# apachepinot/pinot

Hardware: AMD Instinct MI355X
Metric: rows scanned/sec, 1B-row segment filter+groupby (3 predicates, SUM/MAX GROUP BY g1) (higher is better)
Workload: dtype int64; 1 GPU; 1 segment(s) x 1000000000 rows, one per GPU; SELECT g1, SUM(m), MAX(m) FROM gpuBench WHERE c_inv1 IN (0,1,2,3) AND c_inv2 IN (0,1) AND r_int BETWEEN 250000 AND 749999 GROUP BY g1 ORDER BY g1 LIMIT 1000; query=cfg3, parallelism=segment-per-gpu x1, merge=none (1 segment), entries_scanned_in_filter=249990290

## Files before the change

pinot_amd/csrc/pg_kernels_spec.hip:

```cpp
#define PG_WAVES_PER_BLOCK 12
#define PG_KERNEL template <int PG_NOT_INSTANTIATED> static
#include "pg_kernels.hip"

#define SPEC_LOADERS 4
#ifndef SPEC_TILES
#define SPEC_TILES 2
#endif
#ifndef SPEC_SETS
#define SPEC_SETS 2
#endif
#define SPEC_CONSUMERS 8
#define SPEC_OFF_LIN 0u
#define SPEC_OFF_RNG 256u
#define SPEC_OFF_VAL (256u + 2048u)
#define SPEC_OFF_G0 (256u + 2048u + 8192u)
extern "C" const int pg_spec_waves_per_block = PG_WAVES_PER_BLOCK;
extern "C" int pg_spec_stage_bytes(int bits0, int bits1) { return SPEC_TILES * (((int)SPEC_OFF_G0 + bits0 * 256 + 16 + (bits1 > 0 ? bits1 * 256 + 16 : 0) + 15) & ~15); }

DEVFN void spec_barrier() {
  __builtin_amdgcn_fence(__ATOMIC_RELEASE, "workgroup", "local");
  __builtin_amdgcn_s_barrier();
  __builtin_amdgcn_fence(__ATOMIC_ACQUIRE, "workgroup", "local");
}

template <typename T> DEVFN const GAS T* spec_sgpr_ptr(const void* ptr) {
  const uint64_t v = (uint64_t)ptr;
  const uint32_t lo = (uint32_t)__builtin_amdgcn_readfirstlane((int)(uint32_t)v), hi = (uint32_t)__builtin_amdgcn_readfirstlane((int)(uint32_t)(v >> 32));
  return (const GAS T*)(((uint64_t)hi << 32) | (uint64_t)lo);
}

template <int W> struct SpecCol;
template <> struct SpecCol<0> {};
template <> struct SpecCol<32> { u32x4 r[2]; };
template <> struct SpecCol<24> { u32x4 lo; u32x2 hi; };
template <> struct SpecCol<16> { u32x4 lo; };
template <> struct SpecCol<8> { u32x2 hi; };
constexpr uint32_t spec_img_tile_bytes(int W) { return (uint32_t)(PG_WAVE_DOCS / 8) * (uint32_t)W; }
template <int W> DEVFN void spec_load(SpecCol<W>& c, const uint8_t* base, int wt, int w, int lane) {
  if constexpr (W == 32) {
#pragma unroll
    for (int s = 0; s < 2; s++) {
      const uint8_t* row = base + (size_t)wt * (PG_WAVE_DOCS * 4) + (size_t)(4 * s + w) * 1024u;
      c.r[s] = ldnt((const GAS u32x4*)(spec_sgpr_ptr<uint8_t>(row) + (uint32_t)lane * 16u));
    }
  } else if constexpr (W != 0) {
    const uint8_t* tile = base + (size_t)wt * spec_img_tile_bytes(W);
    if constexpr (W >= 16) c.lo = ldnt((const GAS u32x4*)(spec_sgpr_ptr<uint8_t>(tile + (size_t)w * 1024u) + (uint32_t)lane * 16u));
    if constexpr (W != 16) c.hi = ldnt((const GAS u32x2*)(spec_sgpr_ptr<uint8_t>(tile + (W == 24 ? 4096u : 0u) + (size_t)w * 512u) + (uint32_t)lane * 8u));
  }
}
template <int W> DEVFN void spec_unpack(const SpecCol<W>& c, uint32_t (&a)[4], uint32_t (&b)[4]) {
  if constexpr (W == 32) {
    a[0] = bswap32(c.r[0].x); a[1] = bswap32(c.r[0].y); a[2] = bswap32(c.r[0].z); a[3] = bswap32(c.r[0].w);
    b[0] = bswap32(c.r[1].x); b[1] = bswap32(c.r[1].y); b[2] = bswap32(c.r[1].z); b[3] = bswap32(c.r[1].w);
  } else if constexpr (W == 24) {
    a[0] = __builtin_amdgcn_perm(c.hi.x, c.lo.x, 0x0c040100u); a[1] = __builtin_amdgcn_perm(c.hi.x, c.lo.x, 0x0c050302u);
    a[2] = __builtin_amdgcn_perm(c.hi.x, c.lo.y, 0x0c060100u); a[3] = __builtin_amdgcn_perm(c.hi.x, c.lo.y, 0x0c070302u);
    b[0] = __builtin_amdgcn_perm(c.hi.y, c.lo.z, 0x0c040100u); b[1] = __builtin_amdgcn_perm(c.hi.y, c.lo.z, 0x0c050302u);
    b[2] = __builtin_amdgcn_perm(c.hi.y, c.lo.w, 0x0c060100u); b[3] = __builtin_amdgcn_perm(c.hi.y, c.lo.w, 0x0c070302u);
  } else if constexpr (W == 16) {
    a[0] = c.lo.x & 0xFFFFu; a[1] = c.lo.x >> 16; a[2] = c.lo.y & 0xFFFFu; a[3] = c.lo.y >> 16;
    b[0] = c.lo.z & 0xFFFFu; b[1] = c.lo.z >> 16; b[2] = c.lo.w & 0xFFFFu; b[3] = c.lo.w >> 16;
  } else if constexpr (W == 8) {
#pragma unroll
    for (int e = 0; e < 4; e++) { a[e] = (c.hi.x >> (8 * e)) & 0xFFu; b[e] = (c.hi.y >> (8 * e)) & 0xFFu; }
  }
}
template <int SW, int VW> struct SpecTile {
  SpecCol<SW> scan;
  SpecCol<VW> val;
  u32x4 grp;
};
template <int SW, int VW> struct SpecStage { SpecTile<SW, VW> tile[SPEC_TILES]; uint32_t post[8]; uint32_t tail; };
template <int NG> struct SpecQuad {
  uint32_t lin, rng;
  u32x4 val;
  uint32_t win[NG][2];
};

template <int W> struct SpecWidth { static constexpr int value = W; };
template <int NG, bool HAS_INDEX, bool HAS_SCAN, bool HAS_TAIL = false, bool NARROW = false>
__device__ __forceinline__ void spec_body(const PgQueryPlan& p) {
  extern __shared__ __attribute__((aligned(16))) uint64_t smem[];
  __shared__ uint32_t s_stat[PG_MAX_STATS];
  const int t = threadIdx.x;
  const int lane = t & 63;
  const int wave = uniform(t >> 6);
  int64_t* lds_table = reinterpret_cast<int64_t*>(smem);
  if (t < PG_MAX_STATS) s_stat[t] = 0;
  const uint32_t real_slots = (uint32_t)p.n_groups * (uint32_t)p.replicas;
  const uint32_t table_slots = real_slots + 64u;
  for (int o = 0; o < p.n_ops; o++) {
    const int64_t ident = pg_acc_identity(p.ops[o].fn, p.ops[o].is_float);
    for (uint32_t i = t; i < table_slots; i += PG_BLOCK) lds_table[(size_t)o * table_slots + i] = ident;
  }
  const uint32_t bits0 = (uint32_t)p.gcols[0].bits, bits1 = NG > 1 ? (uint32_t)p.gcols[NG - 1].bits : 0u;
  const uint32_t off_g1 = SPEC_OFF_G0 + bits0 * 256u + 16u;
  const uint32_t tile_bytes = (off_g1 + (NG > 1 ? bits1 * 256u + 16u : 0u) + 15u) & ~15u;
  const uint32_t stage_bytes = tile_bytes * SPEC_TILES;
  uint8_t* stage0 = reinterpret_cast<uint8_t*>(smem) + (((size_t)p.n_ops * table_slots * 8u + 15u) & ~(size_t)15u);
  const CAS PgScanLeaf& L = cptr(p.scans)[HAS_SCAN ? p.fast_scan : 0];
  const int grid = (int)gridDim.x;
  const int n_mine = (int)blockIdx.x < p.n_wtiles ? (p.n_wtiles - (int)blockIdx.x + grid - 1) / grid : 0;
  const int n_stages = (n_mine + SPEC_TILES - 1) / SPEC_TILES;
  __syncthreads();

  if (wave < SPEC_LOADERS) {
    const int w = wave;
    const uint8_t* const xdata = p.srcs[p.pipe_src].data;
    const uint8_t* const simg = NARROW ? p.spec_simg : nullptr;
    const uint8_t* const vimg = NARROW ? p.spec_vimg : nullptr;
    const uint32_t img_slo = NARROW ? p.spec_slo : 0u, img_sspan = NARROW ? p.spec_sspan : 0u, img_vmin = NARROW ? (uint32_t)p.spec_vmin : 0u;
    const bool img_sempty = NARROW && p.spec_sempty != 0;
    const int ggi = (w >> 1) < NG ? (w >> 1) : 0;
    const uint8_t* const gdata = p.gcols[ggi].data;
    const uint32_t gbits = (uint32_t)p.gcols[ggi].bits;
    const uint32_t goff = (uint32_t)(w & 1) * 1024u + (uint32_t)lane * 16u;
    const uint32_t geff = (w >> 1) < NG && goff < gbits * 256u ? goff : 0u;
    const uint8_t* dense_ptr[8];
    int dense_group[8];
#pragma unroll
    for (int j = 0; j < 8; j++) { dense_ptr[j] = HAS_INDEX ? p.dense_ptr[j] : nullptr; dense_group[j] = HAS_INDEX ? p.dense_group[j] : 0; }
    const int dense_groups = p.dense_groups, dense_excl = p.dense_excl;
    const uint8_t* const pipe_tail = HAS_TAIL ? p.pipe_tail : nullptr;
    const int num_docs = p.num_docs;
    const bool scan_pushed = p.fast_scan_pushed != 0;
   auto loaders = [&](auto scan_w, auto val_w) __attribute__((always_inline)) {
    constexpr int SW = HAS_SCAN ? decltype(scan_w)::value : 0, VW = decltype(val_w)::value;
    const RangeI32 r32 = !HAS_SCAN ? RangeI32{0, 0u, false} : (SW == 32 ? make_range_i32(L.lo, L.hi) : RangeI32{(int32_t)img_slo, img_sspan, img_sempty});
    const uint8_t* sdata = !HAS_SCAN ? nullptr : (SW == 32 ? L.data : simg);
    const uint8_t* vdata = VW == 32 ? xdata : vimg;
    const uint32_t vmin = VW == 32 ? 0u : img_vmin;
    uint32_t ld_cand = 0;
    auto issue = [&](int sidx, SpecStage<SW, VW>& st) __attribute__((always_inline)) {
#pragma unroll
      for (int tt = 0; tt < SPEC_TILES; tt++) {
        const int i = sidx * SPEC_TILES + tt;
        const int wt = (int)blockIdx.x + (i < n_mine ? i : n_mine - 1) * grid;
        SpecTile<SW, VW>& tl = st.tile[tt];
        __builtin_amdgcn_sched_barrier(0);
        spec_load<SW>(tl.scan, sdata, wt, w, lane);
        spec_load<VW>(tl.val, vdata, wt, w, lane);
        __builtin_amdgcn_sched_barrier(0);
        {
          const uint8_t* base = gdata + (size_t)wt * (size_t)(PG_WAVE_DOCS / 8) * (size_t)gbits;
          tl.grp = ldnt((const GAS u32x4*)(spec_sgpr_ptr<uint8_t>(base) + geff));
        }
        __builtin_amdgcn_sched_barrier(0);
      }
      if (HAS_INDEX) {
        const int i = sidx * SPEC_TILES + (w % SPEC_TILES);
        const int wt = (int)blockIdx.x + (i < n_mine ? i : n_mine - 1) * grid;
#pragma unroll
        for (int j = 0; j < 8; j++) st.post[j] = *(const GAS uint32_t*)(spec_sgpr_ptr<uint8_t>(dense_ptr[j] + (size_t)wt * 256u) + (uint32_t)lane * 4u);
        __builtin_amdgcn_sched_barrier(0);
      }
      if (HAS_TAIL) {
        const int i = sidx * SPEC_TILES + (w % SPEC_TILES);
        const int wt = (int)blockIdx.x + (i < n_mine ? i : n_mine - 1) * grid;
        st.tail = *(const GAS uint32_t*)(spec_sgpr_ptr<uint8_t>(pipe_tail + (size_t)wt * 256u) + (uint32_t)lane * 4u);
        __builtin_amdgcn_sched_barrier(0);
      }
    };
    auto publish = [&](uint8_t* stage, const SpecStage<SW, VW>& st) __attribute__((always_inline)) {
#ifdef PG_SPEC_NO_PUBLISH
      {
        uint32_t acc = 0;
#pragma unroll
        for (int tt = 0; tt < SPEC_TILES; tt++) {
          uint32_t a[4] = {0u, 0u, 0u, 0u}, b[4] = {0u, 0u, 0u, 0u};
          spec_unpack<SW>(st.tile[tt].scan, a, b); acc += a[0] ^ b[3];
          spec_unpack<VW>(st.tile[tt].val, a, b); acc += a[0] ^ b[3];
          acc += st.tile[tt].grp.x;
        }
        if (acc == 0x12345678u) *reinterpret_cast<uint32_t*>(stage) = acc;
        return;
      }
#endif
#pragma unroll
      for (int tt = 0; tt < SPEC_TILES; tt++) {
        uint8_t* buf = stage + (uint32_t)tt * tile_bytes;
        const SpecTile<SW, VW>& tl = st.tile[tt];
        if (HAS_SCAN) {
          uint32_t q[2][4];
          spec_unpack<SW>(tl.scan, q[0], q[1]);
#pragma unroll
          for (int s = 0; s < 2; s++) {
            uint32_t m = (uint32_t)in_range_i32(r32, (int32_t)q[s][0]) | ((uint32_t)in_range_i32(r32, (int32_t)q[s][1]) << 1) |
                         ((uint32_t)in_range_i32(r32, (int32_t)q[s][2]) << 2) | ((uint32_t)in_range_i32(r32, (int32_t)q[s][3]) << 3);
            m = r32.empty ? 0u : m;
            *reinterpret_cast<uint32_t*>(buf + SPEC_OFF_RNG + (uint32_t)(4 * s + w) * 256u + (uint32_t)lane * 4u) = m;
          }
        }
        {
          uint32_t q[2][4];
          spec_unpack<VW>(tl.val, q[0], q[1]);
#pragma unroll
          for (int s = 0; s < 2; s++) {
            u32x4 v;
            v.x = q[s][0] + vmin; v.y = q[s][1] + vmin; v.z = q[s][2] + vmin; v.w = q[s][3] + vmin;
            *reinterpret_cast<u32x4*>(buf + SPEC_OFF_VAL + (uint32_t)(4 * s + w) * 1024u + (uint32_t)lane * 16u) = v;
          }
        }
        *reinterpret_cast<u32x4*>(buf + (ggi == 0 ? SPEC_OFF_G0 : off_g1) + geff) = tl.grp;
      }
    };
    auto publish_lin = [&](uint8_t* stage, const SpecStage<SW, VW>& st, int sidx) __attribute__((always_inline)) {
      if (w >= SPEC_TILES) return;
      const int i = sidx * SPEC_TILES + w;
      const int wt = (int)blockIdx.x + i * grid;
      const int64_t rem = i < n_mine ? (int64_t)num_docs - (int64_t)wt * PG_WAVE_DOCS : 0;
      const int32_t n_valid = rem >= PG_WAVE_DOCS ? PG_WAVE_DOCS : (rem > 0 ? (int32_t)rem : 0);
      uint32_t lin = valid_lin_mask(n_valid, lane);
      if (HAS_INDEX) {
        uint32_t grp[4] = {0u, 0u, 0u, 0u};
#pragma unroll
        for (int j = 0; j < 8; j++) {
          const int gj = dense_group[j];
#pragma unroll
          for (int k = 0; k < 4; k++) grp[k] |= gj == k ? st.post[j] : 0u;
        }
#pragma unroll
        for (int k = 0; k < 4; k++)
          if (k < dense_groups) lin &= ((dense_excl >> k) & 1) ? ~grp[k] : grp[k];
      }
      *reinterpret_cast<uint32_t*>(stage + (uint32_t)w * tile_bytes + SPEC_OFF_LIN + (uint32_t)lane * 4u) = HAS_TAIL ? lin & st.tail : lin;
      ld_cand += (uint32_t)__popc(lin);
    };
    constexpr int SETS = HAS_SCAN ? SPEC_SETS : 2 * SPEC_SETS;
    SpecStage<SW, VW> st[SETS];
    auto buf_of = [&](int sg) __attribute__((always_inline)) { return stage0 + (uint32_t)(sg & 1) * stage_bytes; };
    if (n_stages > 0) {
#pragma unroll
      for (int k = 0; k < SETS; k++) issue(k, st[k]);
    }
    int s = 0;
    for (; s + SETS - 1 < n_stages; s += SETS) {
#pragma unroll
      for (int k = 0; k < SETS; k++) {
        publish(buf_of(s + k), st[k]);
        publish_lin(buf_of(s + k), st[k], s + k);
        issue(s + k + SETS, st[k]);
        spec_barrier();
      }
    }
#pragma unroll
    for (int k = 0; k < SETS - 1; k++)
      if (s + k < n_stages) {
        publish(buf_of(s + k), st[k]);
        publish_lin(buf_of(s + k), st[k], s + k);
        spec_barrier();
      }
    const uint32_t csum = wave_sum_u32(ld_cand);
    if (HAS_SCAN && !scan_pushed && lane == 0 && csum) atomicAdd(&s_stat[L.stat_slot], csum);
   };
    if constexpr (!NARROW) {
      loaders(SpecWidth<32>{}, SpecWidth<32>{});
    } else {
      const int sb = uniform(p.spec_sbits), vb = uniform(p.spec_vbits);
      auto with_scan = [&](auto scan_w) __attribute__((always_inline)) {
        switch (vb) {
          case 8: loaders(scan_w, SpecWidth<8>{}); break;
          case 16: loaders(scan_w, SpecWidth<16>{}); break;
          case 24: loaders(scan_w, SpecWidth<24>{}); break;
          default: loaders(scan_w, SpecWidth<32>{}); break;
        }
      };
      switch (sb) {
        case 8: with_scan(SpecWidth<8>{}); break;
        case 16: with_scan(SpecWidth<16>{}); break;
        case 24: with_scan(SpecWidth<24>{}); break;
        default: with_scan(SpecWidth<32>{}); break;
      }
    }
  } else {
    const int c = wave - SPEC_LOADERS;
    const uint32_t R = (uint32_t)p.replicas;
    const uint32_t rep = (uint32_t)t & (R - 1u);
    const uint32_t stride = table_slots;
    const uint32_t trash_slot = real_slots + (uint32_t)lane;
    const uint32_t q = (uint32_t)c * 64u + (uint32_t)lane;
    const uint32_t nib = ((uint32_t)lane & 7u) * 4u;
    uint32_t my_matched = 0;
    const int n_ops = uniform(p.n_ops);
    uint64_t ops_code = 0;
    for (int o = 0; o < n_ops; o++) {
      const PgAccOp op = p.ops[uniform(o)];
      ops_code |= (uint64_t)(op.src < 0 ? 0u : (op.fn == PG_ACC_SUM ? 1u : (op.fn == PG_ACC_MIN ? 2u : 3u))) << (2 * o);
    }
    ops_code = ((uint64_t)(uint32_t)uniform((int)(uint32_t)(ops_code >> 32)) << 32) | (uint64_t)(uint32_t)uniform((int)(uint32_t)ops_code);
    const int has_out_words = uniform(p.out_words != nullptr ? 1 : 0);
    auto fetch = [&](const uint8_t* buf, SpecQuad<NG>& d) __attribute__((always_inline)) {
      d.lin = *reinterpret_cast<const uint32_t*>(buf + SPEC_OFF_LIN + (q >> 3) * 4u);
      d.rng = HAS_SCAN ? *reinterpret_cast<const uint32_t*>(buf + SPEC_OFF_RNG + q * 4u) : 0xFu;
      d.val = *reinterpret_cast<const u32x4*>(buf + SPEC_OFF_VAL + q * 16u);
#pragma unroll
      for (int gi = 0; gi < NG; gi++) {
        const uint32_t di = __umul24(4u * q, (uint32_t)p.gcols[gi].bits) >> 5;
        const uint32_t* win = reinterpret_cast<const uint32_t*>(buf + (gi == 0 ? SPEC_OFF_G0 : off_g1)) + di;
        d.win[gi][0] = win[0]; d.win[gi][1] = win[1];
      }
    };
    auto aggregate = [&](const SpecQuad<NG> (&d)[SPEC_TILES], int sidx) __attribute__((always_inline)) {
      constexpr int ND = 4 * SPEC_TILES;
      uint32_t slot[ND];
      int32_t v[ND];
#pragma unroll
      for (int tt = 0; tt < SPEC_TILES; tt++) {
        const int i = sidx * SPEC_TILES + tt;
        const uint32_t cand = (d[tt].lin >> nib) & 0xFu;
        const uint32_t m = d[tt].rng & cand;
        my_matched += (uint32_t)__popc(m);
        if (has_out_words && i < n_mine) {
          const int wt = (int)blockIdx.x + i * grid;
          const uint32_t word = or_reduce8(m << nib);
          if ((lane & 7) == 0) reinterpret_cast<uint32_t*>(p.out_words)[(int64_t)wt * 64 + (int64_t)(q >> 3)] = word;
        }
#ifndef PG_SPEC_NO_TABLE
#pragma unroll
        for (int e = 0; e < 4; e++) slot[4 * tt + e] = rep;
#pragma unroll
        for (int gi = 0; gi < NG; gi++) {
          const PgGroupCol& gc = p.gcols[gi];
          const uint32_t bits = (uint32_t)gc.bits, mask = (1u << gc.bits) - 1u;
          const uint32_t mult = (uint32_t)gc.mult * R;
          uint32_t dv[4];
          decode_packed_quad<true>(d[tt].win[gi], q, bits, mask, dv);
#pragma unroll
          for (int e = 0; e < 4; e++) slot[4 * tt + e] += __umul24(dv[e], mult);
        }
#pragma unroll
        for (int e = 0; e < 4; e++) slot[4 * tt + e] = ((m >> e) & 1u) ? slot[4 * tt + e] : trash_slot;
        v[4 * tt + 0] = (int32_t)d[tt].val.x; v[4 * tt + 1] = (int32_t)d[tt].val.y; v[4 * tt + 2] = (int32_t)d[tt].val.z; v[4 * tt + 3] = (int32_t)d[tt].val.w;
#endif
      }
#ifdef PG_SPEC_NO_TABLE
      return;
#endif
      for (int o = 0; o < n_ops; o++) {
        const uint32_t code = (uint32_t)(ops_code >> (2 * o)) & 3u;
        int64_t* base = lds_table + (size_t)o * stride;
        if (code == 0u) {
#pragma unroll
          for (int e = 0; e < ND; e++) atomicAdd(reinterpret_cast<unsigned long long*>(base + slot[e]), 1ULL);
        } else if (code == 1u) {
#pragma unroll
          for (int e = 0; e < ND; e++) atomicAdd(reinterpret_cast<unsigned long long*>(base + slot[e]), (unsigned long long)(int64_t)v[e]);
        } else if (code == 2u) {
#pragma unroll
          for (int e = 0; e < ND; e++) atomicMin(reinterpret_cast<long long*>(base + slot[e]), (long long)v[e]);
        } else {
#pragma unroll
          for (int e = 0; e < ND; e++) atomicMax(reinterpret_cast<long long*>(base + slot[e]), (long long)v[e]);
        }
      }
    };
// ... 84 lines not shown
```

pinot_amd/csrc/pg_segment.cpp:

```cpp
#include <hip/hip_runtime.h>

#include <algorithm>
#include <cmath>

#include "pg_internal.hpp"

extern "C" __global__ void __launch_bounds__(256) pg_column_magnitude_kernel(const uint8_t* __restrict__ data, int64_t n, int val_type,
                                                                             unsigned long long* __restrict__ out) {
  unsigned long long mx = 0, bad = 0;
  for (int64_t i = (int64_t)blockIdx.x * blockDim.x + threadIdx.x; i < n; i += (int64_t)gridDim.x * blockDim.x) {
    unsigned long long a;
    if (val_type == PG_V_I64) {
      const unsigned long long v = __builtin_bswap64(reinterpret_cast<const unsigned long long*>(data)[i]);
      a = (long long)v < 0 ? 0ULL - v : v;
    } else {
      double d;
      if (val_type == PG_V_F32) d = (double)__uint_as_float(__builtin_bswap32(reinterpret_cast<const uint32_t*>(data)[i]));
      else d = __longlong_as_double((long long)__builtin_bswap64(reinterpret_cast<const unsigned long long*>(data)[i]));
      a = (unsigned long long)__double_as_longlong(d) & 0x7FFFFFFFFFFFFFFFULL;
      if (a >= 0x7FF0000000000000ULL) { bad = 1; a = 0; }
    }
    mx = a > mx ? a : mx;
  }
  for (int off = 32; off > 0; off >>= 1) {
    const unsigned long long o = __shfl_xor(mx, off, 64);
    mx = o > mx ? o : mx;
    bad |= __shfl_xor(bad, off, 64);
  }
  if ((threadIdx.x & 63) == 0) {
    if (mx) atomicMax(&out[0], mx);
    if (bad) atomicOr(&out[1], 1ULL);
  }
}

extern "C" __global__ void __launch_bounds__(256) pg_column_int_range_kernel(const uint8_t* __restrict__ data, int64_t n, int val_type,
                                                                             long long* __restrict__ out) {
  long long mn = INT64_MAX, mx = INT64_MIN;
  for (int64_t i = (int64_t)blockIdx.x * blockDim.x + threadIdx.x; i < n; i += (int64_t)gridDim.x * blockDim.x) {
    const long long v = val_type == PG_V_I64 ? (long long)__builtin_bswap64(reinterpret_cast<const unsigned long long*>(data)[i])
                                             : (long long)(int32_t)__builtin_bswap32(reinterpret_cast<const uint32_t*>(data)[i]);
    mn = v < mn ? v : mn;
    mx = v > mx ? v : mx;
  }
  for (int off = 32; off > 0; off >>= 1) {
    const long long a = __shfl_xor(mn, off, 64), b = __shfl_xor(mx, off, 64);
    mn = a < mn ? a : mn;
    mx = b > mx ? b : mx;
  }
  if ((threadIdx.x & 63) == 0 && mn <= mx) {
    atomicMin(&out[0], mn);
    atomicMax(&out[1], mx);
  }
}

extern "C" __global__ void __launch_bounds__(256) pg_column_narrow_image_kernel(const uint8_t* __restrict__ data, uint8_t* __restrict__ img,
                                                                                int64_t n_wtiles, int32_t vmin, int bits) {
  const int64_t n = n_wtiles * 256;
  const int64_t tile_bytes = (int64_t)(PG_WAVE_DOCS / 8) * bits;
  for (int64_t i = (int64_t)blockIdx.x * blockDim.x + threadIdx.x; i < n; i += (int64_t)gridDim.x * blockDim.x) {
    const int64_t wt = i >> 8;
    const int b = (int)(i >> 6) & 3, l = (int)i & 63;
    const uint4 qa = *reinterpret_cast<const uint4*>(data + wt * (PG_WAVE_DOCS * 4) + (int64_t)b * 1024 + l * 16);
    const uint4 qb = *reinterpret_cast<const uint4*>(data + wt * (PG_WAVE_DOCS * 4) + (int64_t)(4 + b) * 1024 + l * 16);
    const uint32_t raw[8] = {qa.x, qa.y, qa.z, qa.w, qb.x, qb.y, qb.z, qb.w};
    uint32_t s[8];
    for (int e = 0; e < 8; e++) s[e] = (__builtin_bswap32(raw[e]) - (uint32_t)vmin) & (bits == 24 ? 0xFFFFFFu : (bits == 16 ? 0xFFFFu : 0xFFu));
    uint8_t* tile = img + wt * tile_bytes;
    if (bits >= 16) {
      uint4 lo;
      lo.x = (s[0] & 0xFFFFu) | (s[1] << 16); lo.y = (s[2] & 0xFFFFu) | (s[3] << 16);
      lo.z = (s[4] & 0xFFFFu) | (s[5] << 16); lo.w = (s[6] & 0xFFFFu) | (s[7] << 16);
      *reinterpret_cast<uint4*>(tile + (int64_t)b * 1024 + l * 16) = lo;
    }
    if (bits != 16) {
      const int sh = bits == 24 ? 16 : 0;
      uint2 hi;
      hi.x = ((s[0] >> sh) & 0xFFu) | (((s[1] >> sh) & 0xFFu) << 8) | (((s[2] >> sh) & 0xFFu) << 16) | (((s[3] >> sh) & 0xFFu) << 24);
      hi.y = ((s[4] >> sh) & 0xFFu) | (((s[5] >> sh) & 0xFFu) << 8) | (((s[6] >> sh) & 0xFFu) << 16) | (((s[7] >> sh) & 0xFFu) << 24);
      *reinterpret_cast<uint2*>(tile + (bits == 24 ? 4096 : 0) + (int64_t)b * 512 + l * 8) = hi;
    }
  }
}

extern "C" __global__ void __launch_bounds__(256) pg_column_max_dict_id_kernel(const uint8_t* __restrict__ data, int64_t n, int bits,
                                                                                unsigned int* __restrict__ out) {
  unsigned int mx = 0;
  const uint64_t mask = (1ULL << bits) - 1ULL;
  for (int64_t i = (int64_t)blockIdx.x * blockDim.x + threadIdx.x; i < n; i += (int64_t)gridDim.x * blockDim.x) {
    const uint64_t bit = (uint64_t)i * (uint64_t)bits;
    const uint8_t* p = data + (bit >> 3);
    uint64_t w = 0;
    for (int k = 0; k < 8; k++) w = (w << 8) | p[k];
    const unsigned int v = (unsigned int)((w >> (64 - bits - (int)(bit & 7))) & mask);
    mx = v > mx ? v : mx;
  }
  for (int off = 32; off > 0; off >>= 1) {
    const unsigned int o = __shfl_xor(mx, off, 64);
    mx = o > mx ? o : mx;
  }
  if ((threadIdx.x & 63) == 0 && mx) atomicMax(out, mx);
}

namespace pg {

static int32_t fx_exp_of(double max_abs) {
  if (!(max_abs > 0)) return 0;
  int e = 0;
  (void)std::frexp(max_abs, &e);
  return (int32_t)(16 * (int)std::floor(((double)e + 15.0) / 16.0));
}

static inline uint32_t be32(const uint8_t* p) {
  return ((uint32_t)p[0] << 24) | ((uint32_t)p[1] << 16) | ((uint32_t)p[2] << 8) | (uint32_t)p[3];
}
static inline uint64_t be64(const uint8_t* p) { return ((uint64_t)be32(p) << 32) | be32(p + 4); }
static inline uint16_t le16(const uint8_t* p) { return (uint16_t)(p[0] | (p[1] << 8)); }
static inline uint32_t le32(const uint8_t* p) {
  return (uint32_t)p[0] | ((uint32_t)p[1] << 8) | ((uint32_t)p[2] << 16) | ((uint32_t)p[3] << 24);
}

Column* Segment::find(const char* n) {
  if (!n) return nullptr;
  auto it = columns.find(n);
  return it == columns.end() ? nullptr : it->second.get();
}

static size_t padded_docs(const Segment& seg) { return (size_t)seg.n_tiles * PG_TILE_DOCS; }

static void check_dict_ids(const Column& c, int64_t n) {
  if (n <= 0 || c.cardinality <= 0 || !(c.bits >= 31 || ((int64_t)1 << c.bits) > (int64_t)c.cardinality)) return;
  DeviceBuffer out(4, true);
  const int grid = (int)std::max<int64_t>(1, std::min<int64_t>(2048, (n + 255) / 256));
  hipLaunchKernelGGL(pg_column_max_dict_id_kernel, dim3(grid), dim3(256), 0, 0, c.fwd_dev.as<uint8_t>(), n, c.bits, out.as<unsigned int>());
  PG_HIP(hipGetLastError());
  unsigned int mx = 0;
  PG_HIP(hipMemcpy(&mx, out.ptr, 4, hipMemcpyDeviceToHost));
  if ((int64_t)mx >= (int64_t)c.cardinality)
    fail(PG_ERR_INVALID_ARGUMENT, "forward index of %s holds dictId %u, the dictionary has %d values", c.name.c_str(), mx, c.cardinality);
}

static void upload_fixed_bit(Segment& seg, Column& c, const uint8_t* src, uint64_t len) {
  uint64_t need = ((uint64_t)seg.total_docs * (uint64_t)c.bits + 7) / 8;
  if (len < need) fail(PG_ERR_INVALID_ARGUMENT, "forward index of %s is %llu bytes, need %llu", c.name.c_str(),
                       (unsigned long long)len, (unsigned long long)need);
  size_t alloc = (padded_docs(seg) * (size_t)c.bits + 7) / 8 + 64;
  c.fwd_dev.alloc(alloc, true);
  c.fwd_dev.upload(src, need);
  c.col_kind = PG_COL_FIXED_BIT;
  c.fwd_bytes_logical = need;
  check_dict_ids(c, (int64_t)seg.total_docs);
}

static void parse_inverted_index(Segment& seg, Column& c, const uint8_t* inv, uint64_t len) {
  const int32_t card = c.cardinality;
  const uint64_t off_end = ((uint64_t)card + 1) * 4;
  if (len < off_end) fail(PG_ERR_INVALID_ARGUMENT, "inverted index of %s too short", c.name.c_str());
  const uint64_t first = be32(inv);
  const uint8_t* bitmap_buffer = inv + off_end;
  c.posting_begin.assign((size_t)card + 1, 0);
  std::vector<uint8_t> staging;
  staging.reserve(len);
  const uint32_t max_key = (uint32_t)((padded_docs(seg) + PG_CHUNK_DOCS - 1) / PG_CHUNK_DOCS);
// ... 693 lines not shown
      offs.resize((size_t)used_chunks + 1);
      decompress_fixed_byte_chunks(compression, fwd, offs, (uint32_t)docs_per_chunk * (uint32_t)width, need, c.fwd_dev.as<uint8_t>(), d.name);
    }
    c.col_kind = width == 4 ? PG_COL_RAW32 : PG_COL_RAW64;
    c.fwd_bytes_logical = need;
  } else {
    fail(PG_ERR_UNSUPPORTED, "column %s: forward index encoding %d", d.name, c.fwd_encoding);
  }

  if (c.has_dictionary && (c.data_type == PG_TYPE_LONG || c.data_type == PG_TYPE_FLOAT || c.data_type == PG_TYPE_DOUBLE)) {
    const uint8_t* dp = c.dict_host.data();
    double mx = 0;
    for (int32_t i = 0; i < c.cardinality; i++) {
      if (c.data_type == PG_TYPE_LONG) {
        const int64_t v = (int64_t)be64(dp + (size_t)i * 8);
        const uint64_t a = v < 0 ? 0ULL - (uint64_t)v : (uint64_t)v;
        c.max_abs_int = std::max(c.max_abs_int, a);
      } else {
        double v;
        if (c.data_type == PG_TYPE_FLOAT) { uint32_t u = be32(dp + (size_t)i * 4); float f; memcpy(&f, &u, 4); v = (double)f; }
        else { uint64_t u = be64(dp + (size_t)i * 8); memcpy(&v, &u, 8); }
        if (std::isfinite(v)) mx = std::max(mx, std::fabs(v));
        else c.has_nonfinite = true;
      }
    }
    c.fx_exp = fx_exp_of(mx);
  } else if (!c.has_dictionary && (c.val_type == PG_V_I64 || c.val_type == PG_V_F32 || c.val_type == PG_V_F64) &&
             (c.col_kind == PG_COL_RAW32 || c.col_kind == PG_COL_RAW64) && seg.total_docs > 0) {
    DeviceBuffer out(16, true);
    hipLaunchKernelGGL(pg_column_magnitude_kernel, dim3(1024), dim3(256), 0, 0, c.fwd_dev.as<uint8_t>(), (int64_t)seg.total_docs, c.val_type,
                       out.as<unsigned long long>());
    PG_HIP(hipGetLastError());
    unsigned long long h[2] = {0, 0};
    PG_HIP(hipMemcpy(h, out.ptr, sizeof(h), hipMemcpyDeviceToHost));
    if (c.val_type == PG_V_I64) c.max_abs_int = h[0];
    else {
      double mx;
      memcpy(&mx, &h[0], 8);
      c.fx_exp = fx_exp_of(mx);
      c.has_nonfinite = h[1] != 0;
    }
  }

  if (!c.has_dictionary && (c.val_type == PG_V_I32 || c.val_type == PG_V_I64) && (c.col_kind == PG_COL_RAW32 || c.col_kind == PG_COL_RAW64) &&
      seg.total_docs > 0) {
    const long long init[2] = {INT64_MAX, INT64_MIN};
    DeviceBuffer out(16);
    out.upload(init, sizeof(init));
    hipLaunchKernelGGL(pg_column_int_range_kernel, dim3(1024), dim3(256), 0, 0, c.fwd_dev.as<uint8_t>(), (int64_t)seg.total_docs, c.val_type,
                       out.as<long long>());
    PG_HIP(hipGetLastError());
    long long h[2] = {0, 0};
    PG_HIP(hipMemcpy(h, out.ptr, sizeof(h), hipMemcpyDeviceToHost));
    if (h[0] <= h[1]) { c.has_int_range = true; c.int_min = h[0]; c.int_max = h[1]; }
  }

  if (d.inverted_index.size > 0 && c.has_dictionary && c.fwd_encoding != PG_FWD_DICT_SORTED)
    parse_inverted_index(seg, c, (const uint8_t*)d.inverted_index.addr, d.inverted_index.size);

  seg.device_bytes += c.fwd_dev.size + c.dict_dev.size + c.containers_dev.size + c.descs_dev.size + c.mv_offsets_dev.size + c.vb_offsets_dev.size;
  seg.columns.emplace(c.name, std::move(col));
}

bool narrow_image_eligible(const Column& c) {
  return !c.has_dictionary && !c.is_mv && !c.raw_mv && c.col_kind == PG_COL_RAW32 && c.val_type == PG_V_I32 && c.has_int_range &&
         c.int_max - c.int_min < ((int64_t)1 << 24);
}

bool narrow_image(Segment& seg, Column& c) {
  std::lock_guard<std::mutex> g(seg.mu);
  if (c.img_state != 0) return c.img_state == 1;
  c.img_state = 2;
  const int64_t n_wtiles = (int64_t)seg.n_tiles * PG_WTILES_PER_TILE;
  if (!narrow_image_eligible(c) || n_wtiles <= 0 || c.fwd_dev.size < (size_t)n_wtiles * (PG_WAVE_DOCS * 4)) return false;
  const int64_t span = c.int_max - c.int_min;
  const int bits = span < 256 ? 8 : (span < 65536 ? 16 : 24);
  void* ptr = nullptr;
  const size_t bytes = (size_t)(n_wtiles * narrow_image_tile_bytes(bits));
  if (hipMalloc(&ptr, bytes) != hipSuccess) {
    (void)hipGetLastError();
    return false;
  }
  c.img_dev.ptr = ptr; c.img_dev.size = bytes; c.img_dev.device = seg.device;
  const int grid = (int)std::min<int64_t>((n_wtiles * 256 + 255) / 256, 8192);
  hipLaunchKernelGGL(pg_column_narrow_image_kernel, dim3(grid), dim3(256), 0, 0, c.fwd_dev.as<uint8_t>(), c.img_dev.as<uint8_t>(), n_wtiles,
                     (int32_t)c.int_min, bits);
  PG_HIP(hipGetLastError());
  PG_HIP(hipDeviceSynchronize());
  c.img_bits = bits;
  c.img_state = 1;
  seg.device_bytes += bytes;
  return true;
}

}
```

Measured before the change: 840.3 billion rows/s.

## Split narrow-image loaders into scan/value role pairs with wider per-lane image layout

Reorganizes the narrow column image so each wave handles half a tile and each lane holds 16 positions in 16-byte rows. Loader waves are specialized by role: two waves load and filter the scan column, two load the value column, with the LIN (posting-list) work done by one role. The aim is to reduce per-wave memory instructions, use full 16-byte loads for 8-bit columns, and spread the loader work more evenly. This adds role-dependent code paths and constrains the path to SPEC_TILES==2 and the indexed-scan shape.

```diff
diff --git a/pinot_amd/csrc/pg_image_layout.h b/pinot_amd/csrc/pg_image_layout.h
--- /dev/null
+++ b/pinot_amd/csrc/pg_image_layout.h
@@ -0,0 +1,19 @@
+#pragma once
+#include <stdint.h>
+
+#define PG_IMG_TILE_DOCS 2048
+#define PG_IMG_ROW_BYTES 1024
+#define PG_IMG_POSITIONS 16
+
+struct PgImgSlot { int half, lane, pos; };
+
+constexpr PgImgSlot pg_img_slot_of_doc(int d) { return PgImgSlot{(d >> 8) & 1, (d >> 2) & 63, 4 * (d >> 9) + (d & 3)}; }
+constexpr int pg_img_quad_row(int half, int pos) { return half + 2 * (pos >> 2); }
+constexpr int pg_img_doc_of_slot(int half, int lane, int pos) { return 4 * (64 * pg_img_quad_row(half, pos) + lane) + (pos & 3); }
+
+constexpr int64_t pg_img_tile_bytes(int bits) { return (int64_t)(PG_IMG_TILE_DOCS / 8) * bits; }
+constexpr uint32_t pg_img_lo_row(int half, int j) { return (uint32_t)(2 * half + j) * PG_IMG_ROW_BYTES; }
+constexpr uint32_t pg_img_hi_row(int bits, int half) { return (bits == 24 ? 4u * PG_IMG_ROW_BYTES : 0u) + (uint32_t)half * PG_IMG_ROW_BYTES; }
+constexpr uint32_t pg_img_raw_row(int half, int k) { return (uint32_t)pg_img_quad_row(half, 4 * k) * PG_IMG_ROW_BYTES; }
+constexpr uint32_t pg_img_lo_offset(int half, int lane, int pos) { return pg_img_lo_row(half, pos >> 3) + (uint32_t)lane * 16u + (uint32_t)(pos & 7) * 2u; }
+constexpr uint32_t pg_img_hi_offset(int bits, int half, int lane, int pos) { return pg_img_hi_row(bits, half) + (uint32_t)lane * 16u + (uint32_t)pos; }
diff --git a/pinot_amd/csrc/pg_kernels_spec.hip b/pinot_amd/csrc/pg_kernels_spec.hip
--- a/pinot_amd/csrc/pg_kernels_spec.hip
+++ b/pinot_amd/csrc/pg_kernels_spec.hip
@@ -1,6 +1,7 @@
 #define PG_WAVES_PER_BLOCK 12
 #define PG_KERNEL template <int PG_NOT_INSTANTIATED> static
 #include "pg_kernels.hip"
+#include "pg_image_layout.h"
 
 #define SPEC_LOADERS 4
 #ifndef SPEC_TILES
@@ -10,6 +11,9 @@
 #define SPEC_SETS 2
 #endif
 #define SPEC_CONSUMERS 8
+#ifndef SPEC_LIN_ROLE
+#define SPEC_LIN_ROLE 1
+#endif
 #define SPEC_OFF_LIN 0u
 #define SPEC_OFF_RNG 256u
 #define SPEC_OFF_VAL (256u + 2048u)
@@ -32,10 +36,6 @@
 template <int W> struct SpecCol;
 template <> struct SpecCol<0> {};
 template <> struct SpecCol<32> { u32x4 r[2]; };
-template <> struct SpecCol<24> { u32x4 lo; u32x2 hi; };
-template <> struct SpecCol<16> { u32x4 lo; };
-template <> struct SpecCol<8> { u32x2 hi; };
-constexpr uint32_t spec_img_tile_bytes(int W) { return (uint32_t)(PG_WAVE_DOCS / 8) * (uint32_t)W; }
 template <int W> DEVFN void spec_load(SpecCol<W>& c, const uint8_t* base, int wt, int w, int lane) {
   if constexpr (W == 32) {
 #pragma unroll
@@ -43,27 +43,40 @@
       const uint8_t* row = base + (size_t)wt * (PG_WAVE_DOCS * 4) + (size_t)(4 * s + w) * 1024u;
       c.r[s] = ldnt((const GAS u32x4*)(spec_sgpr_ptr<uint8_t>(row) + (uint32_t)lane * 16u));
     }
-  } else if constexpr (W != 0) {
-    const uint8_t* tile = base + (size_t)wt * spec_img_tile_bytes(W);
-    if constexpr (W >= 16) c.lo = ldnt((const GAS u32x4*)(spec_sgpr_ptr<uint8_t>(tile + (size_t)w * 1024u) + (uint32_t)lane * 16u));
-    if constexpr (W != 16) c.hi = ldnt((const GAS u32x2*)(spec_sgpr_ptr<uint8_t>(tile + (W == 24 ? 4096u : 0u) + (size_t)w * 512u) + (uint32_t)lane * 8u));
   }
 }
 template <int W> DEVFN void spec_unpack(const SpecCol<W>& c, uint32_t (&a)[4], uint32_t (&b)[4]) {
   if constexpr (W == 32) {
     a[0] = bswap32(c.r[0].x); a[1] = bswap32(c.r[0].y); a[2] = bswap32(c.r[0].z); a[3] = bswap32(c.r[0].w);
     b[0] = bswap32(c.r[1].x); b[1] = bswap32(c.r[1].y); b[2] = bswap32(c.r[1].z); b[3] = bswap32(c.r[1].w);
-  } else if constexpr (W == 24) {
-    a[0] = __builtin_amdgcn_perm(c.hi.x, c.lo.x, 0x0c040100u); a[1] = __builtin_amdgcn_perm(c.hi.x, c.lo.x, 0x0c050302u);
-    a[2] = __builtin_amdgcn_perm(c.hi.x, c.lo.y, 0x0c060100u); a[3] = __builtin_amdgcn_perm(c.hi.x, c.lo.y, 0x0c070302u);
-    b[0] = __builtin_amdgcn_perm(c.hi.y, c.lo.z, 0x0c040100u); b[1] = __builtin_amdgcn_perm(c.hi.y, c.lo.z, 0x0c050302u);
-    b[2] = __builtin_amdgcn_perm(c.hi.y, c.lo.w, 0x0c060100u); b[3] = __builtin_amdgcn_perm(c.hi.y, c.lo.w, 0x0c070302u);
-  } else if constexpr (W == 16) {
-    a[0] = c.lo.x & 0xFFFFu; a[1] = c.lo.x >> 16; a[2] = c.lo.y & 0xFFFFu; a[3] = c.lo.y >> 16;
-    b[0] = c.lo.z & 0xFFFFu; b[1] = c.lo.z >> 16; b[2] = c.lo.w & 0xFFFFu; b[3] = c.lo.w >> 16;
+  }
+}
+static_assert(PG_IMG_TILE_DOCS == PG_WAVE_DOCS, "pg_image_layout.h describes a wave tile");
+template <int W> struct SpecPairCol { u32x4 r[W / 8]; };
+template <int W> DEVFN void spec_pair_load(SpecPairCol<W>& c, const uint8_t* base, int wt, int h, int lane) {
+  const uint8_t* tile = base + (size_t)wt * (size_t)(W == 32 ? PG_WAVE_DOCS * 4 : (int)pg_img_tile_bytes(W));
+#pragma unroll
+  for (int i = 0; i < W / 8; i++) {
+    const uint32_t row = W == 32 ? pg_img_raw_row(h, i) : (W >= 16 && i < 2 ? pg_img_lo_row(h, i) : pg_img_hi_row(W, h));
+    c.r[i] = ldnt((const GAS u32x4*)(spec_sgpr_ptr<uint8_t>(tile + row) + (uint32_t)lane * 16u));
+  }
+}
+template <int W> DEVFN void spec_pair_unpack(const SpecPairCol<W>& c, int k, uint32_t (&q)[4]) {
+  if constexpr (W == 32) {
+#pragma unroll
+    for (int e = 0; e < 4; e++) q[e] = bswap32(c.r[k][e]);
   } else if constexpr (W == 8) {
 #pragma unroll
-    for (int e = 0; e < 4; e++) { a[e] = (c.hi.x >> (8 * e)) & 0xFFu; b[e] = (c.hi.y >> (8 * e)) & 0xFFu; }
+    for (int e = 0; e < 4; e++) q[e] = (c.r[0][k] >> (8 * e)) & 0xFFu;
+  } else {
+    const uint32_t a = c.r[k >> 1][2 * (k & 1)], b = c.r[k >> 1][2 * (k & 1) + 1];
+    if constexpr (W == 24) {
+      const uint32_t hi = c.r[2][k];
+      q[0] = __builtin_amdgcn_perm(hi, a, 0x0c040100u); q[1] = __builtin_amdgcn_perm(hi, a, 0x0c050302u);
+      q[2] = __builtin_amdgcn_perm(hi, b, 0x0c060100u); q[3] = __builtin_amdgcn_perm(hi, b, 0x0c070302u);
+    } else {
+      q[0] = a & 0xFFFFu; q[1] = a >> 16; q[2] = b & 0xFFFFu; q[3] = b >> 16;
+    }
   }
 }
 template <int SW, int VW> struct SpecTile {
@@ -72,6 +85,8 @@
   u32x4 grp;
 };
 template <int SW, int VW> struct SpecStage { SpecTile<SW, VW> tile[SPEC_TILES]; uint32_t post[8]; uint32_t tail; };
+template <int W> struct SpecPairTile { SpecPairCol<W> col; u32x4 grp; };
+template <int W> struct SpecPairStage { SpecPairTile<W> tile[SPEC_TILES]; uint32_t post[8]; uint32_t tail; };
 template <int NG> struct SpecQuad {
   uint32_t lin, rng;
   u32x4 val;
@@ -112,6 +127,7 @@
     const uint8_t* const vimg = NARROW ? p.spec_vimg : nullptr;
     const uint32_t img_slo = NARROW ? p.spec_slo : 0u, img_sspan = NARROW ? p.spec_sspan : 0u, img_vmin = NARROW ? (uint32_t)p.spec_vmin : 0u;
     const bool img_sempty = NARROW && p.spec_sempty != 0;
+    const int img_sbits = NARROW ? uniform(p.spec_sbits) : 32, img_vbits = NARROW ? uniform(p.spec_vbits) : 32;
     const int ggi = (w >> 1) < NG ? (w >> 1) : 0;
     const uint8_t* const gdata = p.gcols[ggi].data;
     const uint32_t gbits = (uint32_t)p.gcols[ggi].bits;
@@ -127,10 +143,10 @@
     const bool scan_pushed = p.fast_scan_pushed != 0;
    auto loaders = [&](auto scan_w, auto val_w) __attribute__((always_inline)) {
     constexpr int SW = HAS_SCAN ? decltype(scan_w)::value : 0, VW = decltype(val_w)::value;
-    const RangeI32 r32 = !HAS_SCAN ? RangeI32{0, 0u, false} : (SW == 32 ? make_range_i32(L.lo, L.hi) : RangeI32{(int32_t)img_slo, img_sspan, img_sempty});
-    const uint8_t* sdata = !HAS_SCAN ? nullptr : (SW == 32 ? L.data : simg);
-    const uint8_t* vdata = VW == 32 ? xdata : vimg;
-    const uint32_t vmin = VW == 32 ? 0u : img_vmin;
+    const RangeI32 r32 = !HAS_SCAN ? RangeI32{0, 0u, false} : make_range_i32(L.lo, L.hi);
+    const uint8_t* sdata = !HAS_SCAN ? nullptr : L.data;
+    const uint8_t* vdata = xdata;
+    const uint32_t vmin = 0u;
     uint32_t ld_cand = 0;
     auto issue = [&](int sidx, SpecStage<SW, VW>& st) __attribute__((always_inline)) {
 #pragma unroll
@@ -254,24 +270,154 @@
     const uint32_t csum = wave_sum_u32(ld_cand);
     if (HAS_SCAN && !scan_pushed && lane == 0 && csum) atomicAdd(&s_stat[L.stat_slot], csum);
    };
+   auto pair_loaders = [&](auto role, auto width) __attribute__((always_inline)) {
+    constexpr int ROLE = decltype(role)::value, W = decltype(width)::value;
+    constexpr bool LIN = ROLE == SPEC_LIN_ROLE;
+    static_assert(SPEC_TILES == 2, "a pair of loaders holds the posting dwords of the stage's two tiles");
+    const int h = w & 1;
+    const RangeI32 r32 = ROLE != 0 ? RangeI32{0, 0u, false} : (W == 32 ? make_range_i32(L.lo, L.hi) : RangeI32{(int32_t)img_slo, img_sspan, img_sempty});
+    const uint8_t* cdata = ROLE == 0 ? (W == 32 ? L.data : simg) : (W == 32 ? xdata : vimg);
+    const uint32_t vmin = W == 32 ? 0u : img_vmin;
+    uint32_t ld_cand = 0;
+    auto issue_tile = [&](int sidx, SpecPairStage<W>& st, int tt) __attribute__((always_inline)) {
+      const int i = sidx * SPEC_TILES + tt;
+      const int wt = (int)blockIdx.x + (i < n_mine ? i : n_mine - 1) * grid;
+      SpecPairTile<W>& tl = st.tile[tt];
+      __builtin_amdgcn_sched_barrier(0);
+      spec_pair_load<W>(tl.col, cdata, wt, h, lane);
+      __builtin_amdgcn_sched_barrier(0);
+      {
+        const uint8_t* base = gdata + (size_t)wt * (size_t)(PG_WAVE_DOCS / 8) * (size_t)gbits;
+        tl.grp = ldnt((const GAS u32x4*)(spec_sgpr_ptr<uint8_t>(base) + geff));
+      }
+      __builtin_amdgcn_sched_barrier(0);
+    };
+    auto issue_post = [&](int sidx, SpecPairStage<W>& st) __attribute__((always_inline)) {
+      {
+        const int i = sidx * SPEC_TILES + h;
+        const int wt = (int)blockIdx.x + (i < n_mine ? i : n_mine - 1) * grid;
+#pragma unroll
+        for (int j = 0; j < 8; j++) st.post[j] = *(const GAS uint32_t*)(spec_sgpr_ptr<uint8_t>(dense_ptr[j] + (size_t)wt * 256u) + (uint32_t)lane * 4u);
+        __builtin_amdgcn_sched_barrier(0);
+        if (HAS_TAIL) {
+          st.tail = *(const GAS uint32_t*)(spec_sgpr_ptr<uint8_t>(pipe_tail + (size_t)wt * 256u) + (uint32_t)lane * 4u);
+          __builtin_amdgcn_sched_barrier(0);
+        }
+      }
+    };
+    auto issue = [&](int sidx, SpecPairStage<W>& st) __attribute__((always_inline)) {
+#pragma unroll
+      for (int tt = 0; tt < SPEC_TILES; tt++) issue_tile(sidx, st, tt);
+      issue_post(sidx, st);
+    };
+    auto publish_tile = [&](uint8_t* stage, const SpecPairStage<W>& st, int tt) __attribute__((always_inline)) {
+#ifdef PG_SPEC_NO_PUBLISH
+      {
+        uint32_t acc = 0;
+#pragma unroll
+        for (int k = 0; k < 4; k++) {
+          uint32_t q[4] = {0u, 0u, 0u, 0u};
+          spec_pair_unpack<W>(st.tile[tt].col, k, q); acc += q[0] ^ q[3];
+        }
+        acc += st.tile[tt].grp.x;
+        if (acc == 0x12345678u) *reinterpret_cast<uint32_t*>(stage) = acc;
+        return;
+      }
+#endif
+      {
+        uint8_t* buf = stage + (uint32_t)tt * tile_bytes;
+        const SpecPairTile<W>& tl = st.tile[tt];
+#pragma unroll
+        for (int k = 0; k < 4; k++) {
+          const uint32_t row = (uint32_t)pg_img_quad_row(h, 4 * k);
+          uint32_t q[4];
+          spec_pair_unpack<W>(tl.col, k, q);
+          if constexpr (ROLE == 0) {
+            uint32_t m = (uint32_t)in_range_i32(r32, (int32_t)q[0]) | ((uint32_t)in_range_i32(r32, (int32_t)q[1]) << 1) |
+                         ((uint32_t)in_range_i32(r32, (int32_t)q[2]) << 2) | ((uint32_t)in_range_i32(r32, (int32_t)q[3]) << 3);
+            m = r32.empty ? 0u : m;
+            *reinterpret_cast<uint32_t*>(buf + SPEC_OFF_RNG + row * 256u + (uint32_t)lane * 4u) = m;
+          } else {
+            u32x4 v;
+            v.x = q[0] + vmin; v.y = q[1] + vmin; v.z = q[2] + vmin; v.w = q[3] + vmin;
+            *reinterpret_cast<u32x4*>(buf + SPEC_OFF_VAL + row * 1024u + (uint32_t)lane * 16u) = v;
+          }
+        }
+        *reinterpret_cast<u32x4*>(buf + (ggi == 0 ? SPEC_OFF_G0 : off_g1) + geff) = tl.grp;
+      }
+    };
+    auto publish = [&](uint8_t* stage, const SpecPairStage<W>& st) __attribute__((always_inline)) {
+#pragma unroll
+      for (int tt = 0; tt < SPEC_TILES; tt++) publish_tile(stage, st, tt);
+    };
+    auto publish_lin = [&](uint8_t* stage, const SpecPairStage<W>& st, int sidx) __attribute__((always_inline)) {
+      if constexpr (LIN) {
+        const int i = sidx * SPEC_TILES + h;
+        const int wt = (int)blockIdx.x + i * grid;
+        const int64_t rem = i < n_mine ? (int64_t)num_docs - (int64_t)wt * PG_WAVE_DOCS : 0;
+        const int32_t n_valid = rem >= PG_WAVE_DOCS ? PG_WAVE_DOCS : (rem > 0 ? (int32_t)rem : 0);
+        uint32_t lin = valid_lin_mask(n_valid, lane);
+        uint32_t grp[4] = {0u, 0u, 0u, 0u};
+#pragma unroll
+        for (int j = 0; j < 8; j++) {
+          const int gj = dense_group[j];
+#pragma unroll
+          for (int k = 0; k < 4; k++) grp[k] |= gj == k ? st.post[j] : 0u;
+        }
+#pragma unroll
+        for (int k = 0; k < 4; k++)
+          if (k < dense_groups) lin &= ((dense_excl >> k) & 1) ? ~grp[k] : grp[k];
+        *reinterpret_cast<uint32_t*>(stage + (uint32_t)h * tile_bytes + SPEC_OFF_LIN + (uint32_t)lane * 4u) = HAS_TAIL ? lin & st.tail : lin;
+        ld_cand += (uint32_t)__popc(lin);
+      }
+    };
+    constexpr int SETS = SPEC_SETS;
+    SpecPairStage<W> st[SETS];
+    auto buf_of = [&](int sg) __attribute__((always_inline)) { return stage0 + (uint32_t)(sg & 1) * stage_bytes; };
+    if (n_stages > 0) {
+#pragma unroll
+      for (int k = 0; k < SETS; k++) issue(k, st[k]);
+    }
+    int s = 0;
+    for (; s + SETS - 1 < n_stages; s += SETS) {
+#pragma unroll
+      for (int k = 0; k < SETS; k++) {
+#pragma unroll
+        for (int tt = 0; tt < SPEC_TILES; tt++) {
+          publish_tile(buf_of(s + k), st[k], tt);
+          issue_tile(s + k + SETS, st[k], tt);
+        }
+        publish_lin(buf_of(s + k), st[k], s + k);
+        issue_post(s + k + SETS, st[k]);
+        spec_barrier();
+      }
+    }
+#pragma unroll
+    for (int k = 0; k < SETS - 1; k++)
+      if (s + k < n_stages) {
+        publish(buf_of(s + k), st[k]);
+        publish_lin(buf_of(s + k), st[k], s + k);
+        spec_barrier();
+      }
+    if constexpr (LIN) {
+      const uint32_t csum = wave_sum_u32(ld_cand);
+      if (!scan_pushed && lane == 0 && csum) atomicAdd(&s_stat[L.stat_slot], csum);
+    }
+   };
     if constexpr (!NARROW) {
       loaders(SpecWidth<32>{}, SpecWidth<32>{});
     } else {
-      const int sb = uniform(p.spec_sbits), vb = uniform(p.spec_vbits);
-      auto with_scan = [&](auto scan_w) __attribute__((always_inline)) {
-        switch (vb) {
-          case 8: loaders(scan_w, SpecWidth<8>{}); break;
-          case 16: loaders(scan_w, SpecWidth<16>{}); break;
-          case 24: loaders(scan_w, SpecWidth<24>{}); break;
-          default: loaders(scan_w, SpecWidth<32>{}); break;
+      static_assert(HAS_INDEX && HAS_SCAN, "the loader pairs are the headline shape's");
+      auto with_role = [&](auto role, int bits) __attribute__((always_inline)) {
+        switch (bits) {
+          case 8: pair_loaders(role, SpecWidth<8>{}); break;
+          case 16: pair_loaders(role, SpecWidth<16>{}); break;
+          case 24: pair_loaders(role, SpecWidth<24>{}); break;
+          default: pair_loaders(role, SpecWidth<32>{}); break;
         }
       };
-      switch (sb) {
-        case 8: with_scan(SpecWidth<8>{}); break;
-        case 16: with_scan(SpecWidth<16>{}); break;
-        case 24: with_scan(SpecWidth<24>{}); break;
-        default: with_scan(SpecWidth<32>{}); break;
-      }
+      if (w < 2) with_role(SpecWidth<0>{}, img_sbits);
+      else with_role(SpecWidth<1>{}, img_vbits);
     }
   } else {
     const int c = wave - SPEC_LOADERS;
diff --git a/pinot_amd/csrc/pg_segment.cpp b/pinot_amd/csrc/pg_segment.cpp
--- a/pinot_amd/csrc/pg_segment.cpp
+++ b/pinot_amd/csrc/pg_segment.cpp
@@ -4,6 +4,7 @@
 #include <cmath>
 
 #include "pg_internal.hpp"
+#include "pg_image_layout.h"
 
 extern "C" __global__ void __launch_bounds__(256) pg_column_magnitude_kernel(const uint8_t* __restrict__ data, int64_t n, int val_type,
                                                                              unsigned long long* __restrict__ out) {
@@ -55,29 +56,37 @@
 
 extern "C" __global__ void __launch_bounds__(256) pg_column_narrow_image_kernel(const uint8_t* __restrict__ data, uint8_t* __restrict__ img,
                                                                                 int64_t n_wtiles, int32_t vmin, int bits) {
-  const int64_t n = n_wtiles * 256;
-  const int64_t tile_bytes = (int64_t)(PG_WAVE_DOCS / 8) * bits;
+  static_assert(PG_IMG_TILE_DOCS == PG_WAVE_DOCS, "pg_image_layout.h describes a wave tile");
+  const int64_t n = n_wtiles * 128;
+  const int64_t tile_bytes = pg_img_tile_bytes(bits);
+  const uint32_t mask = bits == 24 ? 0xFFFFFFu : (bits == 16 ? 0xFFFFu : 0xFFu);
   for (int64_t i = (int64_t)blockIdx.x * blockDim.x + threadIdx.x; i < n; i += (int64_t)gridDim.x * blockDim.x) {
-    const int64_t wt = i >> 8;
-    const int b = (int)(i >> 6) & 3, l = (int)i & 63;
-    const uint4 qa = *reinterpret_cast<const uint4*>(data + wt * (PG_WAVE_DOCS * 4) + (int64_t)b * 1024 + l * 16);
-    const uint4 qb = *reinterpret_cast<const uint4*>(data + wt * (PG_WAVE_DOCS * 4) + (int64_t)(4 + b) * 1024 + l * 16);
-    const uint32_t raw[8] = {qa.x, qa.y, qa.z, qa.w, qb.x, qb.y, qb.z, qb.w};
-    uint32_t s[8];
-    for (int e = 0; e < 8; e++) s[e] = (__builtin_bswap32(raw[e]) - (uint32_t)vmin) & (bits == 24 ? 0xFFFFFFu : (bits == 16 ? 0xFFFFu : 0xFFu));
+    const int64_t wt = i >> 7;
+    const int h = (int)(i >> 6) & 1, l = (int)i & 63;
+    uint32_t s[PG_IMG_POSITIONS];
+    for (int k = 0; k < 4; k++) {
+      const uint4 q = *reinterpret_cast<const uint4*>(data + wt * (PG_WAVE_DOCS * 4) + pg_img_raw_row(h, k) + l * 16);
+      const uint32_t raw[4] = {q.x, q.y, q.z, q.w};
+      for (int e = 0; e < 4; e++) s[4 * k + e] = (__builtin_bswap32(raw[e]) - (uint32_t)vmin) & mask;
+    }
     uint8_t* tile = img + wt * tile_bytes;
     if (bits >= 16) {
-      uint4 lo;
-      lo.x = (s[0] & 0xFFFFu) | (s[1] << 16); lo.y = (s[2] & 0xFFFFu) | (s[3] << 16);
-      lo.z = (s[4] & 0xFFFFu) | (s[5] << 16); lo.w = (s[6] & 0xFFFFu) | (s[7] << 16);
-      *reinterpret_cast<uint4*>(tile + (int64_t)b * 1024 + l * 16) = lo;
+      for (int j = 0; j < 2; j++) {
+        const uint32_t* t = s + 8 * j;
+        uint4 lo;
+        lo.x = (t[0] & 0xFFFFu) | (t[1] << 16); lo.y = (t[2] & 0xFFFFu) | (t[3] << 16);
+        lo.z = (t[4] & 0xFFFFu) | (t[5] << 16); lo.w = (t[6] & 0xFFFFu) | (t[7] << 16);
+        *reinterpret_cast<uint4*>(tile + pg_img_lo_row(h, j) + l * 16) = lo;
+      }
     }
     if (bits != 16) {
       const int sh = bits == 24 ? 16 : 0;
-      uint2 hi;
-      hi.x = ((s[0] >> sh) & 0xFFu) | (((s[1] >> sh) & 0xFFu) << 8) | (((s[2] >> sh) & 0xFFu) << 16) | (((s[3] >> sh) & 0xFFu) << 24);
-      hi.y = ((s[4] >> sh) & 0xFFu) | (((s[5] >> sh) & 0xFFu) << 8) | (((s[6] >> sh) & 0xFFu) << 16) | (((s[7] >> sh) & 0xFFu) << 24);
-      *reinterpret_cast<uint2*>(tile + (bits == 24 ? 4096 : 0) + (int64_t)b * 512 + l * 8) = hi;
+      uint32_t hi[4];
+      for (int k = 0; k < 4; k++) {
+        const uint32_t* t = s + 4 * k;
+        hi[k] = ((t[0] >> sh) & 0xFFu) | (((t[1] >> sh) & 0xFFu) << 8) | (((t[2] >> sh) & 0xFFu) << 16) | (((t[3] >> sh) & 0xFFu) << 24);
+      }
+      *reinterpret_cast<uint4*>(tile + pg_img_hi_row(bits, h) + l * 16) = make_uint4(hi[0], hi[1], hi[2], hi[3]);
     }
   }
 }
@@ -937,7 +946,7 @@
     return false;
   }
   c.img_dev.ptr = ptr; c.img_dev.size = bytes; c.img_dev.device = seg.device;
-  const int grid = (int)std::min<int64_t>((n_wtiles * 256 + 255) / 256, 8192);
+  const int grid = (int)std::min<int64_t>((n_wtiles * 128 + 255) / 256, 8192);
   hipLaunchKernelGGL(pg_column_narrow_image_kernel, dim3(grid), dim3(256), 0, 0, c.fwd_dev.as<uint8_t>(), c.img_dev.as<uint8_t>(), n_wtiles,
                      (int32_t)c.int_min, bits);
   PG_HIP(hipGetLastError());
```

After: 862.7 billion rows/s (median of 6 runs). +2.7%, better.
